# CycloneBoy/pdf_table

Measured on AMD Instinct MI355X. Metric: pages/s, higher is better.
Workload: dtype bf16

## Files before the change

include/pdftable_hip.h:

```cpp
#ifndef PDFTABLE_HIP_H
#define PDFTABLE_HIP_H

#include <stddef.h>
#include <stdint.h>

#ifdef __cplusplus
extern "C" {
#endif

#define PT_OK 0
#define PT_ERR_INVALID 1
#define PT_ERR_HIP 2
#define PT_ERR_STATE 3
#define PT_ERR_FORMAT 4

typedef struct pt_engine pt_engine;
typedef void* pt_stream;

int pt_engine_create(int device_id, pt_engine** out);
void pt_engine_destroy(pt_engine* e);
const char* pt_last_error(void);
int pt_abi_version(void);
int pt_engine_check(pt_engine* e);
int pt_engine_set_lstm_cluster(pt_engine* e, int on);
// ... 121 lines not shown
  int32_t resized_w;
  int32_t img_w;
  int32_t reserved;
  int64_t out_off;
} pt_rec_pp_item;
int pt_rec_pp_preprocess(pt_engine* e, const uint8_t* d_pages_rgb, int n_pages, int h, int w, const pt_rec_line* d_lines,
                         const int64_t* h_crop_px, int n_lines, const pt_rec_pp_item* d_items, int n_items, int img_h,
                         int max_img_w, float* d_out, pt_stream stream);
int pt_rec_pp_preprocess_crops(pt_engine* e, const uint8_t* d_crops_rgb, const pt_rec_line* d_lines, const int64_t* h_crop_px,
                               int n_lines, const pt_rec_pp_item* d_items, int n_items, int img_h, int max_img_w, float* d_out,
                               pt_stream stream);

typedef struct pt_tsr_table {
  double minv[6];
  int32_t page, x0, y0, crop_w, crop_h, reserved;
} pt_tsr_table;

int pt_tsr_preprocess(pt_engine* e, const uint8_t* d_pages_rgb, int n_pages, int ph, int pw, const pt_tsr_table* d_tables,
                      int n, int inp_h, int inp_w, int bgr, uint16_t* d_out_bf16, pt_stream stream);

#define PT_TSR_CS_SMALL 8
#define PT_TSR_CS_FEAT 256
int pt_tsr_forward_net(pt_engine* e, const uint16_t* d_input_bf16, int n, int H, int W, float* d_hm, float* d_st,
                       float* d_wh, float* d_ax, float* d_cr, float* d_reg, pt_stream stream);

int pt_tsr_forward_net_wireless(pt_engine* e, const uint16_t* d_input_bf16, int n, int H, int W, float* d_hm, float* d_st,
                                float* d_wh, float* d_ax, float* d_cr, float* d_reg, pt_stream stream);

#define PT_TSR_MAX_CELLS 3000
int pt_tsr_decode(pt_engine* e, const float* d_hm, const float* d_st, const float* d_wh, const float* d_ax,
                  const float* d_cr, const float* d_reg, int n, int h, int w, int wiz_rev, float vis_thresh,
                  int32_t* d_counts, float* d_dets, float* d_logi, pt_stream stream);

int pt_tsr_forward_decode(pt_engine* e, const uint16_t* d_input_bf16, int n, int in_h, int in_w, int wiz_rev,
                          float vis_thresh, int32_t* d_counts, float* d_dets, float* d_logi, pt_stream stream);

int pt_centernet_forward_net(pt_engine* e, const uint16_t* d_input_bf16, int n, int H, int W, float* d_hm, float* d_v2c, float* d_c2v,
                             float* d_reg, pt_stream stream);

#define PT_CENTERNET_MAX_CELLS 1000
int pt_centernet_decode(pt_engine* e, const float* d_hm, const float* d_v2c, const float* d_c2v, const float* d_reg, int n, int h, int w,
                        const double* d_affine, int32_t* d_counts, float* d_cells, pt_stream stream);

int pt_tsr_process(pt_engine* e, const float* d_logi, const float* d_dets, const int32_t* h_counts, int n_tables,
                   int use_2dpe, float* d_logic, float* d_stacked, pt_stream stream);

int pt_op_conv2d(pt_engine* e, const uint16_t* d_in, int B, int H, int W, int Cin, const uint16_t* d_w_tiled,
                 const float* d_bias, int N, int ks, int stride, uint16_t* d_out, int out_cstride, int out_coff,
                 int rep, int shuffle_cout, const uint16_t* d_res, int res_mode, int relu, int split, int out_lo_off,
                 pt_stream stream);
int pt_op_conv1x1_ex(pt_engine* e, const uint16_t* d_in, int B, int H, int W, int Cin, const uint16_t* d_w_tiled, const float* d_bias,
                     int N, uint16_t* d_out, float* d_out_f32, int out_cstride, int n_valid, const float* d_res_f32, int relu,
                     const int32_t* d_ylimit, pt_stream stream);

int pt_op_dcn(pt_engine* e, const uint16_t* d_in, const float* d_om, int B, int H, int W, int C, const uint16_t* d_w_tiled,
              const float* d_bias, int N, uint16_t* d_out, int relu, int split, pt_stream stream);

int pt_op_dwconvt_up_add(pt_engine* e, const uint16_t* d_in, const float* d_w, const uint16_t* d_add, uint16_t* d_out, int B, int h, int w, int C,
                         int f, int split, pt_stream stream);
int pt_op_dcn_up_add(pt_engine* e, const uint16_t* d_in, const float* d_om, int B, int H, int W, int C, const uint16_t* d_w_tiled,
                     const float* d_bias, int N, uint16_t* d_out, int relu, int split, const uint16_t* d_up_in, int up_h, int up_w,
                     const float* d_up_w, int up_f, pt_stream stream);

int pt_op_stem7x7(pt_engine* e, const uint16_t* d_in, int B, int H, int W, const uint16_t* d_w, const float* d_bias,
                  uint16_t* d_out, int split, pt_stream stream);
int pt_op_maxpool3x3s2(pt_engine* e, const uint16_t* d_in, int B, int H, int W, int C, uint16_t* d_out, int split,
                       pt_stream stream);
int pt_op_db_head_final(pt_engine* e, const uint16_t* d_in, int B, int H, int W, const void* d_w, const float* d_bias,
                        float* d_prob, float* d_logits, int split, pt_stream stream);

int pt_op_dwconv(pt_engine* e, const uint16_t* d_in, int B, int H, int W, int C, const float* d_w_taps, const float* d_bias, int k,
                 int stride, int act, uint16_t* d_out, int split, pt_stream stream);
int pt_op_add(pt_engine* e, const uint16_t* d_a, const uint16_t* d_b, uint16_t* d_out, long long npix, int C, int split, pt_stream stream);
int pt_op_maxpool(pt_engine* e, const uint16_t* d_in, int B, int H, int W, int C, int k, int stride, int pad, uint16_t* d_out,
                  int split, pt_stream stream);
int pt_op_avgpool(pt_engine* e, const uint16_t* d_in, int B, int H, int W, int C, int k, uint16_t* d_out, int split, pt_stream stream);
int pt_op_chan_mean(pt_engine* e, const uint16_t* d_in, int B, int HW, int C, float* d_scratch, uint16_t* d_mean, int split, pt_stream stream);
int pt_op_chan_mean_scratch_floats(int B, int C);
int pt_op_scale_channels(pt_engine* e, const uint16_t* d_in, const uint16_t* d_gate, int B, int HW, int C, uint16_t* d_out,
                         int split, pt_stream stream);
int pt_op_act(pt_engine* e, const uint16_t* d_in, long long n_elems, int kind, float alpha, float beta, uint16_t* d_out, int C, int split,
              pt_stream stream);
int pt_op_copy_channels(pt_engine* e, const uint16_t* d_src, long long npix, int src_cstride, int src_coff, uint16_t* d_dst, int dst_cstride, int dst_coff,
                        int n, pt_stream stream);
int pt_op_upsample_nearest(pt_engine* e, const uint16_t* d_in, int B, int H, int W, int C, int factor, uint16_t* d_out, pt_stream stream);
int pt_op_mul(pt_engine* e, const uint16_t* d_a, const uint16_t* d_b, uint16_t* d_out, long long n_elems, int C, int split, pt_stream stream);
int pt_copy_bytes(pt_engine* e, const void* src, void* dst, long long nbytes, pt_stream stream);
int pt_op_layernorm(pt_engine* e, const uint16_t* d_in, long long rows, int c_pad, int c, const float* d_gamma, const float* d_beta, float eps,
                    uint16_t* d_out, int split, pt_stream stream);
int pt_op_softmax(pt_engine* e, const uint16_t* d_in, long long rows, int c_pad, int c, float* d_out_f32, uint16_t* d_out_bf16, int split, pt_stream stream);
int pt_op_attention(pt_engine* e, const uint16_t* d_qkv, int B, int T, int heads, int d, int qkv_cstride, float scale, uint16_t* d_out, int out_cstride,
                    int split, pt_stream stream);

int pt_op_lstm(pt_engine* e, const uint16_t* d_pregates, int pg_cstride, const uint16_t* d_r_packed, int T, int B, int H, int dirs, int reverse,
               uint16_t* d_y, int y_cstride, int split, pt_stream stream);
int pt_op_lstm_packed_elems(int H, int dirs, int split);

int pt_op_conv2d_rect(pt_engine* e, const uint16_t* d_in, int B, int H, int W, int Cin, const uint16_t* d_w_tiled, const float* d_bias, int N, int kh,
                      int kw, int sh, int sw, uint16_t* d_out, int out_cstride, int out_coff, int act, int split, int out_lo_off, pt_stream stream);
int pt_op_dwconv_rect(pt_engine* e, const uint16_t* d_in, int B, int H, int W, int C, const float* d_w_taps, const float* d_bias, int k, int sh, int sw,
                      int act, uint16_t* d_out, int split, pt_stream stream);
int pt_op_pool_rect(pt_engine* e, const uint16_t* d_in, int B, int H, int W, int C, int kind, int kh, int kw, uint16_t* d_out, int split,
                    pt_stream stream);

int pt_op_affine_act(pt_engine* e, const uint16_t* d_in, long long npix, int Cpad, int C, const float* d_s1, const float* d_b1, const float* d_s2,
                     const float* d_b2, int act, uint16_t* d_out, int split, pt_stream stream);
// ... 61 lines not shown
```

pdf_table_amd/csrc/c_api.hip:

```cpp
#include <stdarg.h>
#include <stdio.h>
#include <stdlib.h>

#include <cmath>

#include "common.h"

namespace PT_FMT_NS {
namespace api {

static int ensure(void** buf, size_t* cap, size_t need);

int pt_engine_check(pt_engine* e) {
  PT_REQUIRE(e, "pt_engine_check: null engine");
  if (e->lstm_err && *e->lstm_err) {
    *e->lstm_err = 0;
    e->lstm_cluster = 0;
    pt_set_error("lstm_cluster_kernel: a workgroup waited > 2^22 polls for its peers -- the launch was not co-resident "
                 "(GPU shared with another process or stream?).  The recognition results since the last check are invalid; "
                 "this engine now uses the streaming LSTM kernel (pt_engine_set_lstm_cluster(e, 0)): run the batch again");
    return PT_ERR_HIP;
  }
  return PT_OK;
}
// ... 880 lines not shown

int pt_cls_forward_lines_direct(pt_engine* e, int slot, const uint8_t* d_pages_rgb, int n_pages, int h, int w, const pt_rec_line* d_lines,
                                int n_lines, int max_crop_h, int max_crop_w, int out_h, int out_w, int textline, float* d_logits,
                                int* n_classes, pt_stream stream) {
  PT_REQUIRE(e && d_pages_rgb && d_lines && d_logits && n_lines > 0 && n_pages > 0 && h > 0 && w > 0,
             "pt_cls_forward_lines_direct: bad arguments");
  PT_HIP_CHECK(hipSetDevice(e->device));
  hipStream_t s = reinterpret_cast<hipStream_t>(stream);
  int rc;
  if ((rc = cls_lut(e)) != PT_OK) return rc;
  const int mb = cls_microbatch(), x3 = pt_split(e);
  const size_t per = (size_t)out_h * out_w * (x3 ? 8 : 4);
  const int cap = mb < n_lines ? mb : n_lines;
  if ((rc = ensure(&e->cls_direct_in, &e->cls_direct_in_cap, (size_t)cap * per * sizeof(bf16_t))) != PT_OK) return rc;
  bf16_t* xin = reinterpret_cast<bf16_t*>(e->cls_direct_in);
  for (int i0 = 0; i0 < n_lines; i0 += mb) {
    const int nb = (n_lines - i0) < mb ? (n_lines - i0) : mb;
    {
      PtProfScope ps(e, s, PT_PROF_OTHER, 0, "cls line resize+norm");
      rc = pt_launch_cls_line_resize_norm(d_pages_rgb, h, w, d_lines + i0, nb, max_crop_h, max_crop_w, out_h, out_w, e->cls_lut, x3, xin, s);
      if (rc != PT_OK) return rc;
    }
    rc = pt_pplcnet_forward_net(e, slot, xin, nb, out_h, out_w, textline, d_logits + (size_t)i0 * PT_CLS_MAX_CLASSES, n_classes, s,
                                PT_ARENA_CLS);
    if (rc != PT_OK) return rc;
  }
  return PT_OK;
}

int pt_op_conv2d(pt_engine* e, const uint16_t* d_in, int B, int H, int W, int Cin, const uint16_t* d_w_tiled,
                 const float* d_bias, int N, int ks, int stride, uint16_t* d_out, int out_cstride, int out_coff,
                 int rep, int shuffle_cout, const uint16_t* d_res, int res_mode, int relu, int split, int out_lo_off,
                 pt_stream stream) {
  PT_REQUIRE(e != nullptr, "pt_op_conv2d: null engine");
  ConvDesc d;
  d.in = d_in; d.B = B; d.H = H; d.W = W; d.Cin = Cin; d.w = d_w_tiled; d.bias = d_bias; d.N = N; d.ks = ks;
  d.stride = stride; d.out = d_out; d.out_cstride = out_cstride; d.out_coff = out_coff; d.rep = rep;
  d.shuffle_cout = shuffle_cout; d.res = d_res; d.res_mode = res_mode; d.relu = relu;
  d.split = split; d.out_lo_off = out_lo_off;
  return pt_launch_conv(e, d, reinterpret_cast<hipStream_t>(stream));
}

int pt_op_conv1x1_ex(pt_engine* e, const uint16_t* d_in, int B, int H, int W, int Cin, const uint16_t* d_w_tiled, const float* d_bias,
                     int N, uint16_t* d_out, float* d_out_f32, int out_cstride, int n_valid, const float* d_res_f32, int relu,
                     const int32_t* d_ylimit, pt_stream stream) {
  PT_REQUIRE(e != nullptr, "pt_op_conv1x1_ex: null engine");
  ConvDesc d;
  d.in = d_in; d.B = B; d.H = H; d.W = W; d.Cin = Cin; d.w = d_w_tiled; d.bias = d_bias; d.N = N; d.ks = 1; d.stride = 1;
  d.out = d_out_f32 ? nullptr : d_out; d.out_f32 = d_out_f32; d.out_cstride = out_cstride; d.n_valid = n_valid; d.res_f32 = d_res_f32;
  d.relu = relu; d.ylimit = d_ylimit;
  return pt_launch_conv(e, d, reinterpret_cast<hipStream_t>(stream));
}

int pt_op_stem7x7(pt_engine* e, const uint16_t* d_in, int B, int H, int W, const uint16_t* d_w, const float* d_bias,
                  uint16_t* d_out, int split, pt_stream stream) {
  PT_REQUIRE(e != nullptr, "pt_op_stem7x7: null engine");
  return pt_launch_stem7x7(e, d_in, B, H, W, d_w, d_bias, d_out, split, reinterpret_cast<hipStream_t>(stream));
}

int pt_op_maxpool3x3s2(pt_engine* e, const uint16_t* d_in, int B, int H, int W, int C, uint16_t* d_out, int split,
                       pt_stream stream) {
  PT_REQUIRE(e && d_in && d_out, "pt_op_maxpool3x3s2: bad arguments");
  return pt_launch_maxpool3x3s2(d_in, B, H, W, C, d_out, split, reinterpret_cast<hipStream_t>(stream));
}

int pt_op_db_head_final(pt_engine* e, const uint16_t* d_in, int B, int H, int W, const void* d_w, const float* d_bias,
                        float* d_prob, float* d_logits, int split, pt_stream stream) {
  PT_REQUIRE(e && d_in && d_w && d_bias && (d_prob || d_logits), "pt_op_db_head_final: bad arguments");
  return pt_launch_db_head_final(d_in, B, H, W, d_w, d_bias, d_prob, d_logits, split, reinterpret_cast<hipStream_t>(stream));
}

int pt_op_dcn(pt_engine* e, const uint16_t* d_in, const float* d_om, int B, int H, int W, int C, const uint16_t* d_w_tiled,
              const float* d_bias, int N, uint16_t* d_out, int relu, int split, pt_stream stream) {
  PT_REQUIRE(e && d_in && d_om && d_w_tiled && d_bias && d_out, "pt_op_dcn: null argument");
  PT_REQUIRE(B > 0 && H > 0 && W > 0, "pt_op_dcn: empty map (B=%d H=%d W=%d)", B, H, W);
  return pt_launch_dcn_fused(e, d_in, d_om, d_w_tiled, d_bias, d_out, B, H, W, C, N, split, relu, reinterpret_cast<hipStream_t>(stream));
}

int pt_op_dwconvt_up_add(pt_engine* e, const uint16_t* d_in, const float* d_w, const uint16_t* d_add, uint16_t* d_out, int B, int h, int w, int C,
                         int f, int split, pt_stream stream) {
  PT_REQUIRE(e && d_in && d_w && d_out, "pt_op_dwconvt_up_add: null argument");
  PT_REQUIRE(B > 0 && h > 0 && w > 0 && C > 0, "pt_op_dwconvt_up_add: empty map (B=%d h=%d w=%d C=%d)", B, h, w, C);
  return pt_launch_dwconvt_up_add(d_in, d_w, d_add, d_out, B, h, w, C, f, split, reinterpret_cast<hipStream_t>(stream));
}

int pt_op_dcn_up_add(pt_engine* e, const uint16_t* d_in, const float* d_om, int B, int H, int W, int C, const uint16_t* d_w_tiled,
                     const float* d_bias, int N, uint16_t* d_out, int relu, int split, const uint16_t* d_up_in, int up_h, int up_w,
                     const float* d_up_w, int up_f, pt_stream stream) {
  PT_REQUIRE(e && d_in && d_om && d_w_tiled && d_bias && d_out && d_up_in && d_up_w, "pt_op_dcn_up_add: null argument");
  PT_REQUIRE(B > 0 && H > 0 && W > 0, "pt_op_dcn_up_add: empty map (B=%d H=%d W=%d)", B, H, W);
  PT_REQUIRE(split == 0, "pt_op_dcn_up_add: the (hi | lo) modes keep the two launches (pt_op_dcn, pt_op_dwconvt_up_add)");
  PT_REQUIRE((up_f == 2 || up_f == 4) && up_h > 0 && up_w > 0 && up_h * up_f == H && up_w * up_f == W,
             "pt_op_dcn_up_add: a %dx%d map times %d is not the %dx%d output", up_h, up_w, up_f, H, W);
  return pt_launch_dcn_fused(e, d_in, d_om, d_w_tiled, d_bias, d_out, B, H, W, C, N, split, relu, reinterpret_cast<hipStream_t>(stream), nullptr, nullptr,
                             d_up_in, d_up_w, up_f);
}

int pt_profile_enable(pt_engine* e, int on) {
  PT_REQUIRE(e != nullptr, "pt_profile_enable: null engine");
  PT_REQUIRE(on >= 0 && on < 2 + PT_PROF_NCLASS, "pt_profile_enable: mode %d out of range", on);
  if (on && !e->prof.h_lims)
    PT_HIP_CHECK(hipHostMalloc(reinterpret_cast<void**>(&e->prof.h_lims), PtProfile::MAX_LIMS * sizeof(int), hipHostMallocDefault));
  e->prof.on = on;
  return PT_OK;
}

// ... 75 lines not shown
```

pdf_table_amd/csrc/rec_kernels.hip:

```cpp
#include <math.h>

#include "common.h"

namespace PT_FMT_NS {

typedef __attribute__((ext_vector_type(8))) __bf16 bf16x8;
typedef __attribute__((ext_vector_type(16))) float f32x16;
typedef __attribute__((ext_vector_type(4))) uint32_t u32x4;
typedef __attribute__((ext_vector_type(2))) uint32_t u32x2;

__device__ __forceinline__ float rbf2f(uint32_t bits16) { return a16_to_f32(bits16); }
__device__ __forceinline__ uint32_t rf2bf(float f) { return f32_to_a16(f); }

__global__ __launch_bounds__(256) void rec_warp_kernel(const uint8_t* __restrict__ pages, int ph, int pw,
                                                        const pt_rec_line* __restrict__ lines, int n_lines,
                                                        const long long* __restrict__ pix_off, uint8_t* __restrict__ crops) {
  a16_kernel_enter();
  const int li = blockIdx.y;
  if (li >= n_lines) return;
  const pt_rec_line L = lines[li];
  const int cw = L.crop_w, chh = L.crop_h;
  const long long npx = (long long)cw * chh;
  uint8_t* dst = crops + pix_off[li] * 3;
  const uint8_t* src = pages + (size_t)L.page * ph * pw * 3;
// ... 1847 lines not shown
    hipLaunchKernelGGL((gemm_argmax_kernel<32, 0, 8>), dim3((unsigned)((M + 255) / 256)), dim3(512), SMEM, s, A, M, W3, bias, N, ids, rowmax, nullptr, 0,
                       nullptr, 2 * K, wts);
  }
  if (cls_dma())
    hipLaunchKernelGGL(cls_argmax_dma_kernel<1>, dim3((unsigned)((M + 255) / 256)), dim3(512), CLS_DMA_SMEM, s, A, M, W3, bias, N, nullptr, nullptr, 2 * K, wts,
                       reinterpret_cast<const float*>(wmax), rowmax, cand);
  else
    hipLaunchKernelGGL((gemm_cand_kernel<32>), dim3((unsigned)((M + 127) / 128)), dim3(256), SMEM, s, A, M, 2 * K, W3, wts, bias, N,
                       reinterpret_cast<const float*>(wmax), rowmax, cand);
  hipLaunchKernelGGL(cand_eval_kernel, dim3((unsigned)((M + 15) / 16)), dim3(256), 0, s, A, M, 2 * K, K, W3, bias, N, n_real, cand, ids, maxv, ovf_count,
                     ovf_rows);
  hipLaunchKernelGGL(cand_full_kernel, dim3(2048), dim3(256), 0, s, A, 2 * K, K, W3, bias, n_real, ovf_count, ovf_rows, ids, maxv);
  PT_HIP_CHECK(hipGetLastError());
  return PT_OK;
}

static int gemm_nw(int dflt) {
  static int nw = -1;
  if (nw < 0) {
    const char* ev = getenv("PT_GEMM_NW");
    nw = ev ? (atoi(ev) == 8 ? 8 : 4) : 0;
  }
  return nw ? nw : dflt;
}

int pt_launch_gemm_argmax(const bf16_t* A, long long M, int K, const bf16_t* W, const float* bias, int N, int* ids, float* maxv,
                          hipStream_t s) {
  if ((K != 512 && K != 192) || N % 64 != 0 || M <= 0) return PT_ERR_INVALID;
  constexpr int SMEM = 64 * (512 * 2 + 16) + 64 * 4;
  static bool attr_done = false;
  if (!attr_done) {
    PT_HIP_CHECK(hipFuncSetAttribute(reinterpret_cast<const void*>(&gemm_argmax_kernel<32, 0>), hipFuncAttributeMaxDynamicSharedMemorySize, SMEM));
    PT_HIP_CHECK(hipFuncSetAttribute(reinterpret_cast<const void*>(&gemm_argmax_kernel<12, 0>), hipFuncAttributeMaxDynamicSharedMemorySize, SMEM));
    PT_HIP_CHECK(hipFuncSetAttribute(reinterpret_cast<const void*>(&gemm_argmax_kernel<32, 0, 8>), hipFuncAttributeMaxDynamicSharedMemorySize, SMEM));
    PT_HIP_CHECK(hipFuncSetAttribute(reinterpret_cast<const void*>(&gemm_argmax_kernel<12, 0, 8>), hipFuncAttributeMaxDynamicSharedMemorySize, SMEM));
    attr_done = true;
  }
  const int nw = gemm_nw(K == 512 ? 8 : 4);
  const dim3 grid((unsigned)((M + nw * 32 - 1) / (nw * 32))), blk(nw * 64);
  if (K == 192) {
    if (nw == 8) hipLaunchKernelGGL((gemm_argmax_kernel<12, 0, 8>), grid, blk, 64 * (192 * 2 + 16) + 64 * 4, s, A, M, W, bias, N, ids, maxv, nullptr, 0, nullptr, 192, 6ll * 2048);
    else hipLaunchKernelGGL((gemm_argmax_kernel<12, 0>), grid, blk, 64 * (192 * 2 + 16) + 64 * 4, s, A, M, W, bias, N, ids, maxv, nullptr, 0, nullptr, 192, 6ll * 2048);
  } else {
    if (nw == 8 && cls_dma()) {
      if (cls_dma_attr() != PT_OK) return PT_ERR_HIP;
      hipLaunchKernelGGL(cls_argmax_dma_kernel<0>, grid, blk, CLS_DMA_SMEM, s, A, M, W, bias, N, ids, maxv, 512, 16ll * 2048, nullptr, nullptr, nullptr);
    } else if (nw == 8) hipLaunchKernelGGL((gemm_argmax_kernel<32, 0, 8>), grid, blk, SMEM, s, A, M, W, bias, N, ids, maxv, nullptr, 0, nullptr, 512, 16ll * 2048);
    else hipLaunchKernelGGL((gemm_argmax_kernel<32, 0>), grid, blk, SMEM, s, A, M, W, bias, N, ids, maxv, nullptr, 0, nullptr, 512, 16ll * 2048);
  }
  PT_HIP_CHECK(hipGetLastError());
  return PT_OK;
}

int pt_launch_gemm_rows(const bf16_t* A, long long M, int K, const bf16_t* W, const float* bias, int N, bf16_t* out, int relu,
                        hipStream_t s, const int* tlim) {
  if ((K != 512 && K != 256) || N % 64 != 0 || M <= 0) return PT_ERR_INVALID;
  const int nw = gemm_nw(4);
  const int smem = 64 * (K * 2 + 16) + 64 * 4 + nw * 32 * 80;
  static bool attr_done = false;
  if (!attr_done) {
    PT_HIP_CHECK(hipFuncSetAttribute(reinterpret_cast<const void*>(&gemm_argmax_kernel<32, 1>), hipFuncAttributeMaxDynamicSharedMemorySize, 64 * (512 * 2 + 16) + 256 + 4 * 32 * 80));
    PT_HIP_CHECK(hipFuncSetAttribute(reinterpret_cast<const void*>(&gemm_argmax_kernel<32, 1, 8>), hipFuncAttributeMaxDynamicSharedMemorySize, 64 * (512 * 2 + 16) + 256 + 8 * 32 * 80));
    attr_done = true;
  }
  const dim3 grid((unsigned)((M + nw * 32 - 1) / (nw * 32))), blk(nw * 64);
  if (K == 512) {
    if (nw == 8) hipLaunchKernelGGL((gemm_argmax_kernel<32, 1, 8>), grid, blk, smem, s, A, M, W, bias, N, nullptr, nullptr, out, relu, tlim, 512, 16ll * 2048);
    else hipLaunchKernelGGL((gemm_argmax_kernel<32, 1>), grid, blk, smem, s, A, M, W, bias, N, nullptr, nullptr, out, relu, tlim, 512, 16ll * 2048);
  } else {
    if (nw == 8) hipLaunchKernelGGL((gemm_argmax_kernel<16, 1, 8>), grid, blk, smem, s, A, M, W, bias, N, nullptr, nullptr, out, relu, tlim, 256, 8ll * 2048);
    else hipLaunchKernelGGL((gemm_argmax_kernel<16, 1>), grid, blk, smem, s, A, M, W, bias, N, nullptr, nullptr, out, relu, tlim, 256, 8ll * 2048);
  }
  PT_HIP_CHECK(hipGetLastError());
  return PT_OK;
}

template <int KSTEPS>
__global__ __launch_bounds__(256, KSTEPS == 32 ? 1 : 2) void gemm_rows_x3_kernel(const bf16_t* __restrict__ A, long long M, const bf16_t* __restrict__ W3,
                                                                                 const float* __restrict__ bias, int N, bf16_t* __restrict__ out, int relu,
                                                                                 const int* __restrict__ tlim) {
  a16_kernel_enter();
  constexpr int K = KSTEPS * 16, NCH = K / 32, P = K * 2 + 16;
  constexpr int NPF = NCH;
  extern __shared__ __attribute__((aligned(16))) char smem[];
  char* sw = smem;
  float* sb = reinterpret_cast<float*>(smem + 64 * P);
  const int tid = threadIdx.x, lane = tid & 63, wave = tid >> 6;
  const int lx = lane & 31, q = lane >> 5;
  long long row0 = ((long long)blockIdx.x * 4 + wave) * 32;
  bool live = row0 < M;
  if (tlim) {
    const int total = tlim[0], g = blockIdx.x * 4 + wave;
    if ((int)blockIdx.x * 4 >= total) return;
    live = g < total;
    row0 = live ? (long long)tlim[1 + g] * 32 : 0;
  }
  const long long row = row0 + lx;
  const long long rc = row < M ? row : M - 1;
  bf16x8 ahi[KSTEPS], alo[KSTEPS];
#pragma unroll
  for (int ks = 0; ks < KSTEPS; ++ks) {
    ahi[ks] = *reinterpret_cast<const bf16x8*>(A + rc * (2 * K) + ks * 16 + q * 8);
    alo[ks] = *reinterpret_cast<const bf16x8*>(A + rc * (2 * K) + K + ks * 16 + q * 8);
  }
  u32x4 pf[NPF];
  float pb = 0.f;
  auto prefetch = [&](int st) {
    const bf16_t* wt = W3 + (size_t)(st >> 1) * (3 * NCH * 2048) + (st & 1) * (32 * 32);
#pragma unroll
    for (int j = 0; j < NPF; ++j) {
      const int idx = tid + j * 256, plane = idx / (NCH * 128), rem = idx - plane * (NCH * 128), c = rem >> 7, rp = rem & 127;
      pf[j] = *reinterpret_cast<const u32x4*>(wt + (size_t)(plane * 2 * NCH + c) * 2048 + rp * 8);
    }
    if (tid < 32) pb = bias[st * 32 + tid];
  };
  auto commit = [&]() {
// ... 95 lines not shown
```

pdf_table_amd/engine.py:

```python
from __future__ import annotations

import contextlib
import ctypes as C
import functools
import threading
from typing import Optional, Sequence, Tuple

import numpy as np
import torch

from . import lib as L

__all__ = ["HipEngine", "REC_LINE_DTYPE", "CLS_IMAGE_DTYPE", "REC_PP_ITEM_DTYPE"]

TSR_TABLE_DTYPE = np.dtype([("minv", "<f8", (6,)), ("page", "<i4"), ("x0", "<i4"), ("y0", "<i4"),
                            ("crop_w", "<i4"), ("crop_h", "<i4"), ("reserved", "<i4")])
CLS_IMAGE_DTYPE = np.dtype([("offset", "<i8"), ("h", "<i4"), ("w", "<i4")])
REC_LINE_DTYPE = np.dtype([("minv", np.float64, (9,)), ("page", np.int32), ("crop_w", np.int32), ("crop_h", np.int32),
                           ("reserved", np.int32)])


REC_PP_ITEM_DTYPE = np.dtype([("line", "<i4"), ("resized_w", "<i4"), ("img_w", "<i4"), ("reserved", "<i4"),
                              ("out_off", "<i8")])

# ... 576 lines not shown
        T, Tc = cfg["max_len"] + 1, cfg["max_len_cell"] + 1
        tag = torch.zeros((n, T, cfg["num_classes"]), dtype=torch.float32, device=self._tdev)
        box = torch.zeros((n, T, 4), dtype=torch.float32, device=self._tdev)
        lens = np.zeros(n, np.int32)
        counts = np.zeros(n, np.int32)
        ip = lambda a: a.ctypes.data_as(C.POINTER(C.c_int))
        L.check(self.lib.pt_tsr_mtl_structure(self._h, _ptr(f3), n, hw, _ptr(tag), _ptr(box), ip(lens), ip(counts), 1 if force_redecode else 0,
                                              self._stream()), "pt_tsr_mtl_structure")
        total = int(counts.sum())
        steps = np.zeros(n, np.int32)
        ids = torch.zeros((max(total, 1), Tc), dtype=torch.int32, device=self._tdev)
        prob = torch.zeros((max(total, 1), Tc), dtype=torch.float32, device=self._tdev)
        logits = torch.zeros((max(total, 1), Tc, cfg["num_classes_cell"]), dtype=torch.float32, device=self._tdev) if want_cell_logits else None
        L.check(self.lib.pt_tsr_mtl_cells(self._h, total, _ptr(ids), _ptr(prob), _ptr(logits), ip(steps), 1 if force_redecode else 0, self._stream()),
                "pt_tsr_mtl_cells")
        return dict(tag_logits=tag, boxes=box, lens=lens, cell_counts=counts, cell_steps=steps, cell_ids=ids[:total], cell_prob=prob[:total],
                    cell_logits=None if logits is None else logits[:total], cfg=cfg)

    def op_conv2d(self, x: torch.Tensor, w_tiled: torch.Tensor, bias: torch.Tensor, ks: int, stride: int = 1,
                  relu: bool = False, res: Optional[torch.Tensor] = None, res_mode: int = 0, rep: int = 1,
                  shuffle_cout: int = 0, out: Optional[torch.Tensor] = None, out_coff: int = 0,
                  split: int = 0) -> torch.Tensor:
        self._chk(x, self.act_dtype, "x")
        self._chk(bias, torch.float32, "bias")
        B, H, W, Cin = x.shape
        m = 2 if split else 1
        Cin //= m
        N = bias.numel()
        pad = ks // 2
        Ho, Wo = (H + 2 * pad - ks) // stride + 1, (W + 2 * pad - ks) // stride + 1
        if out is None:
            if shuffle_cout:
                out = torch.empty((B, 2 * Ho, 2 * Wo, shuffle_cout * m), dtype=self.act_dtype, device=self._tdev)
            else:
                out = torch.empty((B, Ho * rep, Wo * rep, N * m), dtype=self.act_dtype, device=self._tdev)
        L.check(self.lib.pt_op_conv2d(self._h, _ptr(x), B, H, W, Cin, _ptr(w_tiled), _ptr(bias), N, ks, stride,
                                      _ptr(out), out.shape[-1], out_coff, rep, shuffle_cout, _ptr(res), res_mode,
                                      int(relu), int(split), out.shape[-1] // 2, self._stream()), "pt_op_conv2d")
        return out

    def op_conv1x1_ex(self, x: torch.Tensor, w_tiled: torch.Tensor, bias: torch.Tensor, relu: int = 0, out_f32: bool = False,
                      n_valid: int = 0, res_f32: Optional[torch.Tensor] = None, ylimit: Optional[torch.Tensor] = None) -> torch.Tensor:
        self._chk(x, self.act_dtype, "x")
        self._chk(bias, torch.float32, "bias")
        B, H, W, Cin = x.shape
        N = bias.numel()
        cs = n_valid or N
        out = torch.zeros((B, H, W, cs), dtype=torch.float32 if out_f32 else self.act_dtype, device=self._tdev)
        L.check(self.lib.pt_op_conv1x1_ex(self._h, _ptr(x), B, H, W, Cin, _ptr(w_tiled), _ptr(bias), N, None if out_f32 else _ptr(out),
                                          _ptr(out) if out_f32 else None, cs, n_valid, _ptr(res_f32), int(relu), _ptr(ylimit),
                                          self._stream()), "pt_op_conv1x1_ex")
        return out

    def op_dcn(self, x: torch.Tensor, om: torch.Tensor, w_tiled: torch.Tensor, bias: torch.Tensor, relu: bool = True, split: int = 0) -> torch.Tensor:
        self._chk(x, self.act_dtype, "x")
        self._chk(om, torch.float32, "om")
        self._chk(bias, torch.float32, "bias")
        B, H, W, Cc = x.shape
        m = 2 if split else 1
        Cc //= m
        if tuple(om.shape) != (B, H, W, 32):
            raise ValueError(f"op_dcn: om must be [B,H,W,32], got {tuple(om.shape)}")
        N = bias.numel()
        out = torch.empty((B, H, W, N * m), dtype=self.act_dtype, device=self._tdev)
        L.check(self.lib.pt_op_dcn(self._h, _ptr(x), _ptr(om), B, H, W, Cc, _ptr(w_tiled), _ptr(bias), N, _ptr(out), int(relu), int(split),
                                   self._stream()), "pt_op_dcn")
        return out

    def op_dwconvt_up_add(self, x: torch.Tensor, w_taps: torch.Tensor, add: Optional[torch.Tensor], f: int, split: int = 0) -> torch.Tensor:
        self._chk(x, self.act_dtype, "x")
        self._chk(w_taps, torch.float32, "w_taps")
        B, h, w, Cc = x.shape
        if add is not None:
            self._chk(add, self.act_dtype, "add")
            if tuple(add.shape) != (B, h * f, w * f, Cc):
                raise ValueError(f"op_dwconvt_up_add: add must be {(B, h * f, w * f, Cc)}, got {tuple(add.shape)}")
        out = torch.empty((B, h * f, w * f, Cc), dtype=self.act_dtype, device=self._tdev)
        L.check(self.lib.pt_op_dwconvt_up_add(self._h, _ptr(x), _ptr(w_taps), _ptr(add), _ptr(out), B, h, w, Cc // 2 if split else Cc, int(f),
                                              int(split), self._stream()), "pt_op_dwconvt_up_add")
        return out

    def op_dcn_up_add(self, x: torch.Tensor, om: torch.Tensor, w_tiled: torch.Tensor, bias: torch.Tensor, up_in: torch.Tensor, up_taps: torch.Tensor,
                      f: int, relu: bool = True, split: int = 0) -> torch.Tensor:
        self._chk(x, self.act_dtype, "x")
        self._chk(om, torch.float32, "om")
        self._chk(bias, torch.float32, "bias")
        self._chk(up_in, self.act_dtype, "up_in")
        self._chk(up_taps, torch.float32, "up_taps")
        B, H, W, Cc = x.shape
        if tuple(om.shape) != (B, H, W, 32):
            raise ValueError(f"op_dcn_up_add: om must be [B,H,W,32], got {tuple(om.shape)}")
        N = bias.numel()
        if up_in.dim() != 4 or up_in.shape[0] != B or up_in.shape[3] != N:
            raise ValueError(f"op_dcn_up_add: up_in must be [{B},h,w,{N}], got {tuple(up_in.shape)}")
        out = torch.empty((B, H, W, N), dtype=self.act_dtype, device=self._tdev)
        L.check(self.lib.pt_op_dcn_up_add(self._h, _ptr(x), _ptr(om), B, H, W, Cc // 2 if split else Cc, _ptr(w_tiled), _ptr(bias), N, _ptr(out), int(relu),
                                          int(split), _ptr(up_in), up_in.shape[1], up_in.shape[2], _ptr(up_taps), int(f), self._stream()),
                "pt_op_dcn_up_add")
        return out

    def op_dwconv(self, x: torch.Tensor, w_taps: torch.Tensor, bias: torch.Tensor, k: int, stride: int = 1, act: int = 0, split: bool = False) -> torch.Tensor:
        self._chk(x, self.act_dtype, "x")
        self._chk(w_taps, torch.float32, "w_taps")
        self._chk(bias, torch.float32, "bias")
        B, H, W, Cc = x.shape
        pad = k // 2
# ... 341 lines not shown
```

pdf_table_amd/lib.py:

```python
from __future__ import annotations

import ctypes as C
import os

_HERE = os.path.dirname(os.path.abspath(__file__))
LIB_PATH = os.environ.get("PT_LIB_PATH") or os.path.join(_HERE, "libpdftable_hip.so")

PT_MODEL_DB_RESNET18 = 1
PT_MODEL_CRNN = 2
PT_MODEL_LORE_DLA34 = 3
PT_MODEL_LORE_PROCESSOR = 4
PT_MODEL_PICODET = 5
PT_MODEL_LORE_RESNET18 = 6
PT_MODEL_DB_NAS = 7
PT_MODEL_PPLCNET = 8
PT_MODEL_CONVNEXT_VIT = 16
PT_MODEL_MTL_BACKBONE = 17
PT_MODEL_MTL_DECODER = 18
PT_MODEL_CENTERNET_DLA34 = 19
PT_CVIT_W, PT_CVIT_CHUNK_W, PT_CVIT_CHUNK_STEP, PT_CVIT_T, PT_CVIT_NCLS = 804, 300, 252, 201, 7644
PT_CLS_SLOTS = 4
PT_CLS_MAX_CLASSES = 16
PT_LAYOUT_HEAD_CS, PT_LAYOUT_CAND_FLOATS = 40, 48
PT_DET_PRE_DB_PP = 0
# ... 36 lines not shown
        "pt_weights_load_device": (i, [vp, i, vp, sz, vp]),
        "pt_det_plan": (i, [i, i, i, ip, ip]),
        "pt_det_forward": (i, [vp, vp, i, i, i, i, f, i, vp, vp, vp]),
        "pt_det_forward_net": (i, [vp, vp, i, i, i, vp, vp, vp]),
        "pt_det_preprocess": (i, [vp, vp, i, i, i, i, vp, vp]),
        "pt_det_bitmap": (i, [vp, vp, i, i, i, f, i, vp, vp]),
        "pt_det_box_scores": (i, [vp, vp, i, i, i, vp, i, vp, vp]),
        "pt_db_candidates": (i, [vp, i, i, i, f, vp, vp, i, ip]),
        "pt_db_finalize": (i, [vp, vp, i, f, f, f, i, i, i, i, i, vp, vp, i, ip]),
        "pt_db_candidates_batch": (i, [vp, i, i, i, i, f, i, vp, vp, i, vp]),
        "pt_db_finalize_batch": (i, [vp, vp, vp, i, i, f, f, f, i, i, i, i, i, i, i, vp, vp, vp, vp]),
        "pt_rec_forward": (i, [vp, vp, i, i, i, vp, vp, i, vp, vp, vp]),
        "pt_rec_forward_crops": (i, [vp, vp, vp, vp, i, vp, vp, vp]),
        "pt_rec_forward_net": (i, [vp, vp, i, vp, vp, vp]),
        "pt_rec_preprocess": (i, [vp, vp, i, i, i, vp, vp, i, vp, vp]),
        "pt_rec_cvit_forward": (i, [vp, vp, i, i, i, vp, vp, vp, i, vp, vp, vp]),
        "pt_rec_cvit_forward_crops": (i, [vp, vp, vp, vp, vp, i, vp, vp, vp]),
        "pt_rec_cvit_forward_net": (i, [vp, vp, i, i, vp, vp, vp, vp]),
        "pt_rec_cvit_preprocess_crops": (i, [vp, vp, vp, vp, i, vp, vp]),
        "pt_tsr_mtl_backbone_net": (i, [vp, vp, i, i, i, vp, vp]),
        "pt_tsr_mtl_preprocess": (i, [vp, vp, i, i, i, vp, i, i, vp, vp]),
        "pt_tsr_mtl_resized_size": (None, [i, i, i, ip, ip]),
        "pt_tsr_mtl_decoder_config": (i, [vp, ip]),
        "pt_tsr_mtl_structure": (i, [vp, vp, i, i, vp, vp, ip, ip, i, vp]),
        "pt_tsr_mtl_cells": (i, [vp, i, vp, vp, vp, ip, i, vp]),
        "pt_rec_pp_preprocess": (i, [vp, vp, i, i, i, vp, vp, i, vp, i, i, i, vp, vp]),
        "pt_rec_pp_preprocess_crops": (i, [vp, vp, vp, vp, i, vp, i, i, i, vp, vp]),
        "pt_layout_plan": (i, [i, i, ip, ip]),
        "pt_layout_preprocess": (i, [vp, vp, i, i, i, i, i, vp, vp]),
        "pt_layout_forward_net": (i, [vp, vp, i, i, i, vp, vp, vp, vp, vp]),
        "pt_layout_candidates": (i, [vp, vp, vp, vp, vp, i, i, i, i, f, i, vp, vp, vp]),
        "pt_layout_forward": (i, [vp, vp, i, i, i, i, i, i, f, i, vp, vp, vp]),
        "pt_tsr_preprocess": (i, [vp, vp, i, i, i, vp, i, i, i, i, vp, vp]),
        "pt_tsr_forward_net": (i, [vp, vp, i, i, i, vp, vp, vp, vp, vp, vp, vp]),
        "pt_tsr_forward_net_wireless": (i, [vp, vp, i, i, i, vp, vp, vp, vp, vp, vp, vp]),
        "pt_tsr_decode": (i, [vp, vp, vp, vp, vp, vp, vp, i, i, i, i, f, vp, vp, vp, vp]),
        "pt_tsr_forward_decode": (i, [vp, vp, i, i, i, i, f, vp, vp, vp, vp]),
        "pt_tsr_process": (i, [vp, vp, vp, vp, i, i, vp, vp, vp]),
        "pt_centernet_forward_net": (i, [vp, vp, i, i, i, vp, vp, vp, vp, vp]),
        "pt_centernet_decode": (i, [vp, vp, vp, vp, vp, i, i, i, vp, vp, vp, vp]),
        "pt_hard_nms": (i, [vp, vp, vp, i, C.c_double, i, vp, vp]),
        "pt_page_line_mask": (i, [vp, i, i, i, vp, vp]),
        "pt_page_line_angles": (i, [vp, i, i, i, i, i, vp, i, vp]),
        "pt_page_warp_cubic": (i, [vp, i, i, i, vp, vp, i, vp, vp]),
        "pt_page_quarter_turn": (i, [vp, i, i, i, i, vp, vp]),
        "pt_page_pre_tables": (i, [vp, vp]),
        "pt_cls_preprocess": (i, [vp, vp, vp, i, i, i, i, i, vp, vp]),
        "pt_cls_forward_net": (i, [vp, i, vp, i, i, i, i, vp, ip, vp]),
        "pt_cls_forward": (i, [vp, i, vp, vp, i, i, i, i, i, i, vp, ip, vp]),
        "pt_cls_forward_lines": (i, [vp, i, vp, i, i, i, vp, vp, i, i, i, i, i, i, vp, ip, vp]),
        "pt_cls_forward_lines_direct": (i, [vp, i, vp, i, i, i, vp, i, i, i, i, i, i, vp, ip, vp]),
        "pt_op_conv2d": (i, [vp, vp, i, i, i, i, vp, vp, i, i, i, vp, i, i, i, i, vp, i, i, i, i, vp]),
        "pt_op_conv1x1_ex": (i, [vp, vp, i, i, i, i, vp, vp, i, vp, vp, i, i, vp, i, vp, vp]),
        "pt_op_dcn": (i, [vp, vp, vp, i, i, i, i, vp, vp, i, vp, i, i, vp]),
        "pt_op_dwconvt_up_add": (i, [vp, vp, vp, vp, vp, i, i, i, i, i, i, vp]),
        "pt_op_dcn_up_add": (i, [vp, vp, vp, i, i, i, i, vp, vp, i, vp, i, i, vp, i, i, vp, i, vp]),
        "pt_op_stem7x7": (i, [vp, vp, i, i, i, vp, vp, vp, i, vp]),
        "pt_op_maxpool3x3s2": (i, [vp, vp, i, i, i, i, vp, i, vp]),
        "pt_op_db_head_final": (i, [vp, vp, i, i, i, vp, vp, vp, vp, i, vp]),
        "pt_op_dwconv": (i, [vp, vp, i, i, i, i, vp, vp, i, i, i, vp, i, vp]),
        "pt_op_add": (i, [vp, vp, vp, vp, C.c_longlong, i, i, vp]),
        "pt_op_maxpool": (i, [vp, vp, i, i, i, i, i, i, i, vp, i, vp]),
        "pt_op_avgpool": (i, [vp, vp, i, i, i, i, i, vp, i, vp]),
        "pt_op_chan_mean": (i, [vp, vp, i, i, i, vp, vp, i, vp]),
        "pt_op_chan_mean_scratch_floats": (i, [i, i]),
        "pt_op_scale_channels": (i, [vp, vp, vp, i, i, i, vp, i, vp]),
        "pt_op_act": (i, [vp, vp, C.c_longlong, i, C.c_float, C.c_float, vp, i, i, vp]),
        "pt_op_copy_channels": (i, [vp, vp, C.c_longlong, i, i, vp, i, i, i, vp]),
        "pt_op_upsample_nearest": (i, [vp, vp, i, i, i, i, i, vp, vp]),
        "pt_op_mul": (i, [vp, vp, vp, vp, C.c_longlong, i, i, vp]),
        "pt_copy_bytes": (i, [vp, vp, vp, C.c_longlong, vp]),
        "pt_op_layernorm": (i, [vp, vp, C.c_longlong, i, i, vp, vp, C.c_float, vp, i, vp]),
        "pt_op_softmax": (i, [vp, vp, C.c_longlong, i, i, vp, vp, i, vp]),
        "pt_op_attention": (i, [vp, vp, i, i, i, i, i, C.c_float, vp, i, i, vp]),
        "pt_op_lstm": (i, [vp, vp, i, vp, i, i, i, i, i, vp, i, i, vp]),
        "pt_op_lstm_packed_elems": (i, [i, i, i]),
        "pt_op_conv2d_rect": (i, [vp, vp, i, i, i, i, vp, vp, i, i, i, i, i, vp, i, i, i, i, i, vp]),
        "pt_op_dwconv_rect": (i, [vp, vp, i, i, i, i, vp, vp, i, i, i, i, vp, i, vp]),
        "pt_op_pool_rect": (i, [vp, vp, i, i, i, i, i, i, i, vp, i, vp]),
        "pt_op_affine_act": (i, [vp, vp, C.c_longlong, i, i, vp, vp, vp, vp, i, vp, i, vp]),
        "pt_op_db_tail": (i, [vp, vp, i, i, i, i, i, i, vp, vp, vp, vp, vp, i, vp]),
        "pt_profile_enable": (i, [vp, i]),
        "pt_profile_read": (i, [vp, vp, vp, vp]),
        "pt_profile_read_labels": (i, [vp, C.c_char_p, i]),
    }
    for name, (res, args) in P.items():
        try:
            fn = getattr(lib, name)
        except AttributeError:
            raise PtError(f"{LIB_PATH} does not export {name}: it was built from older sources; rebuild it (`python -m pdf_table_amd.build --force`)") from None
        fn.restype = res
        fn.argtypes = args
    return P


EXPORTS = None


def load():
    global _lib, EXPORTS
    if _lib is None:
        import torch
        if not os.path.exists(LIB_PATH):
            raise PtError(f"{LIB_PATH} not found: run `python -m pdf_table_amd.build` (hipcc, gfx950). "
                          "There is no CPU fallback.")
        lib = C.CDLL(LIB_PATH, mode=C.RTLD_GLOBAL)
# ... 14 lines not shown
```

Measured before the change: 787.6.

## Add DMA-pipelined K=256 row GEMM kernel with LDS-staged weight tiles

Adds a new rows_dma_kernel for K=256 row GEMMs that keeps A rows in registers, streams 64-column weight tiles into LDS with buffer_load_lds DMA double-buffering, and interleaves MFMA with the next tile's loads using scheduling barriers. Outputs go through an LDS transpose tile so each store is a coalesced 128-bit buffer store. It is enabled by default unless PT_ROWS_DMA=0, and a pt_op_gemm_rows C/Python entry point is exposed for it. The aim is to hide weight-fetch latency and raise MFMA utilization. In exchange it needs large LDS and runs one 512-thread block per CU, which could limit occupancy.

```diff
diff --git a/include/pdftable_hip.h b/include/pdftable_hip.h
--- a/include/pdftable_hip.h
+++ b/include/pdftable_hip.h
@@ -197,6 +197,9 @@
 int pt_op_conv1x1_ex(pt_engine* e, const uint16_t* d_in, int B, int H, int W, int Cin, const uint16_t* d_w_tiled, const float* d_bias,
                      int N, uint16_t* d_out, float* d_out_f32, int out_cstride, int n_valid, const float* d_res_f32, int relu,
                      const int32_t* d_ylimit, pt_stream stream);
+
+int pt_op_gemm_rows(pt_engine* e, const uint16_t* d_a, long long M, int K, const uint16_t* d_w_tiled, const float* d_bias, int N,
+                    uint16_t* d_out, int relu, const int32_t* d_live, pt_stream stream);
 
 int pt_op_dcn(pt_engine* e, const uint16_t* d_in, const float* d_om, int B, int H, int W, int C, const uint16_t* d_w_tiled,
               const float* d_bias, int N, uint16_t* d_out, int relu, int split, pt_stream stream);
diff --git a/pdf_table_amd/csrc/c_api.hip b/pdf_table_amd/csrc/c_api.hip
--- a/pdf_table_amd/csrc/c_api.hip
+++ b/pdf_table_amd/csrc/c_api.hip
@@ -956,6 +956,14 @@
   return pt_launch_conv(e, d, reinterpret_cast<hipStream_t>(stream));
 }
 
+int pt_op_gemm_rows(pt_engine* e, const uint16_t* d_a, long long M, int K, const uint16_t* d_w_tiled, const float* d_bias, int N,
+                    uint16_t* d_out, int relu, const int32_t* d_live, pt_stream stream) {
+  PT_REQUIRE(e != nullptr, "pt_op_gemm_rows: null engine");
+  PT_REQUIRE(e->precision == PT_PRECISION_BF16 || e->precision == PT_PRECISION_F16, "pt_op_gemm_rows: single-pass precisions only");
+  PT_REQUIRE(relu == 0 || relu == 1 || relu == 4, "pt_op_gemm_rows: relu must be 0, 1 or 4");
+  return pt_launch_gemm_rows(d_a, M, K, d_w_tiled, d_bias, N, d_out, relu, reinterpret_cast<hipStream_t>(stream), d_live);
+}
+
 int pt_op_stem7x7(pt_engine* e, const uint16_t* d_in, int B, int H, int W, const uint16_t* d_w, const float* d_bias,
                   uint16_t* d_out, int split, pt_stream stream) {
   PT_REQUIRE(e != nullptr, "pt_op_stem7x7: null engine");
diff --git a/pdf_table_amd/csrc/rec_kernels.hip b/pdf_table_amd/csrc/rec_kernels.hip
--- a/pdf_table_amd/csrc/rec_kernels.hip
+++ b/pdf_table_amd/csrc/rec_kernels.hip
@@ -1923,6 +1923,165 @@
   return PT_OK;
 }
 
+template <int ACT>
+__device__ __forceinline__ void rows_tile_to_lds(const f32x16& acc, const float* bs, char* dst) {
+#pragma unroll
+  for (int rg = 0; rg < 4; ++rg) {
+    const a16_f32x4 b4 = *reinterpret_cast<const a16_f32x4*>(bs + rg * 8);
+    uint32_t hb[4];
+#pragma unroll
+    for (int k = 0; k < 4; ++k) {
+      float v = acc[rg * 4 + k] + b4[k];
+      if (ACT == 1) v = fmaxf(v, 0.f);
+      else if (ACT == 4) v = gelu_poly(v);
+      hb[k] = rf2bf(v);
+    }
+    *reinterpret_cast<u32x2*>(dst + rg * 16) = u32x2{hb[0] | (hb[1] << 16), hb[2] | (hb[3] << 16)};
+  }
+}
+
+constexpr int ROWS_DMA_SMEM = 2 * 32 * (1024 + 16) + 2 * 64 * 4 + 8 * 32 * 144;
+
+__global__ __launch_bounds__(512, 1) void rows_dma_kernel(const bf16_t* __restrict__ A, long long M, const bf16_t* __restrict__ W,
+                                                          const float* __restrict__ bias, int N, bf16_t* __restrict__ out, int relu,
+                                                          const int* __restrict__ tlim) {
+#if defined(__HIP_DEVICE_COMPILE__)
+  a16_kernel_enter();
+  constexpr int NW = 8, KSTEPS = 16, K = 256, BLK = 1024 + 16, TILE = 32 * BLK, D = 2;
+  constexpr int NDMA = 32 / NW, EVERY = 2 * KSTEPS / NDMA;
+  constexpr int TP = 128 + 16;
+  extern __shared__ __attribute__((aligned(16))) char smem[];
+  float* sb = reinterpret_cast<float*>(smem + 2 * TILE);
+  const int tid = threadIdx.x, lane = tid & 63;
+  const int wave = __builtin_amdgcn_readfirstlane(tid >> 6);
+  const int lx = lane & 31, q = lane >> 5;
+  char* tile = smem + 2 * TILE + 512 + wave * (32 * TP);
+  const long long g0 = ((long long)blockIdx.x * NW + wave) * 2;
+  long long row0[2];
+  bool live[2];
+  if (tlim) {
+    const int total = tlim[0];
+    if ((long long)blockIdx.x * NW * 2 >= total) return;
+#pragma unroll
+    for (int i = 0; i < 2; ++i) {
+      live[i] = g0 + i < total;
+      row0[i] = live[i] ? (long long)tlim[1 + g0 + i] * 32 : 0;
+    }
+  } else {
+#pragma unroll
+    for (int i = 0; i < 2; ++i) {
+      row0[i] = (g0 + i) * 32;
+      live[i] = row0[i] < M;
+    }
+  }
+  bf16x8 areg[2][KSTEPS];
+#pragma unroll
+  for (int i = 0; i < 2; ++i) {
+    const long long row = row0[i] + lx;
+    const long long rc = row < M ? row : M - 1;
+#pragma unroll
+    for (int ks = 0; ks < KSTEPS; ++ks) areg[i][ks] = *reinterpret_cast<const bf16x8*>(A + rc * K + ks * 16 + q * 8);
+  }
+  constexpr int OOB = 0x7FFFF000;
+  const __amdgpu_buffer_rsrc_t r_w = __builtin_amdgcn_make_buffer_rsrc(const_cast<bf16_t*>(W), 0, OOB, 0x00020000);
+  int voff[NDMA];
+  {
+    const int i = lane >> 5, p = (lane & 31) ^ (8 * i);
+#pragma unroll
+    for (int s = 0; s < NDMA; ++s) voff[s] = ((((p >> 2) * 64 + 2 * (wave + NW * s) + i) * 32) + (p & 3) * 8) * 2;
+  }
+  const int fbase = (lx >> 1) * BLK + (lx & 1) * 512 + q * 16;
+  const int fa = fbase + (lx & 1) * 128, fb = fbase - (lx & 1) * 128;
+  const int NT = N / 64;
+#pragma unroll
+  for (int s = 0; s < NDMA; ++s)
+    __builtin_amdgcn_raw_ptr_buffer_load_lds(r_w, (__attribute__((address_space(3))) void*)(smem + (wave + NW * s) * BLK), 16, voff[s], 0, 0, 0);
+  if (tid < 64) sb[tid] = bias[tid];
+  float pb = tid < 64 ? bias[(NT > 1 ? 64 : 0) + tid] : 0.f;
+#pragma unroll
+  for (int i = 0; i < 2; ++i)
+#pragma unroll
+    for (int ks = 0; ks < KSTEPS; ++ks) asm volatile("" : "+v"(areg[i][ks]));
+  __amdgpu_buffer_rsrc_t r_o[2];
+#pragma unroll
+  for (int i = 0; i < 2; ++i) {
+    const long long left = M - row0[i];
+    const int nrec = !live[i] || left <= 0 ? 0 : (int)(left < 32 ? left : 32) * N * 2;
+    r_o[i] = __builtin_amdgcn_make_buffer_rsrc(out + row0[i] * N, 0, __builtin_amdgcn_readfirstlane(nrec), 0x00020000);
+  }
+  constexpr int NST = 8;
+  asm volatile("s_waitcnt vmcnt(0)" ::: "memory");
+  for (int t = 0; t < NT; ++t) {
+    const int b = t & 1;
+    __syncthreads();
+    const bool more = t + 1 < NT;
+    const int soff = more ? (t + 1) * (K * 64 * 2) : 0;
+    if (tid < 64) {
+      sb[(b ^ 1) * 64 + tid] = pb;
+      pb = bias[(t + 2 < NT ? t + 2 : t) * 64 + tid];
+    }
+    const float* sbt = sb + b * 64;
+    f32x16 acc[2][2];
+#pragma unroll
+    for (int half = 0; half < 2; ++half) {
+      const char* wa = smem + b * TILE + half * 16 * BLK + fa;
+      const char* wb = smem + b * TILE + half * 16 * BLK + fb;
+#pragma unroll
+      for (int r = 0; r < 16; ++r) { acc[half][0][r] = 0.f; acc[half][1][r] = 0.f; }
+      bf16x8 f[D + 1];
+#pragma unroll
+      for (int d = 0; d < D; ++d) f[d] = *reinterpret_cast<const bf16x8*>(wa + d * 32);
+#pragma unroll
+      for (int ks = 0; ks < KSTEPS; ++ks) {
+        if (ks + D < KSTEPS) f[(ks + D) % (D + 1)] = *reinterpret_cast<const bf16x8*>((((ks + D) & 4) ? wb : wa) + (ks + D) * 32);
+        acc[half][0] = mfma_32x32x16_a16(f[ks % (D + 1)], areg[0][ks], acc[half][0]);
+        acc[half][1] = mfma_32x32x16_a16(f[ks % (D + 1)], areg[1][ks], acc[half][1]);
+        if ((half * KSTEPS + ks) % EVERY == 0) {
+          const int s = (half * KSTEPS + ks) / EVERY;
+          __builtin_amdgcn_raw_ptr_buffer_load_lds(r_w, (__attribute__((address_space(3))) void*)(smem + (b ^ 1) * TILE + (wave + NW * s) * BLK), 16,
+                                                   more ? voff[s] : OOB, soff, 0, 0);
+        }
+      }
+      __builtin_amdgcn_sched_group_barrier(0x100, D, 0);
+#pragma unroll
+      for (int ks = 0; ks < KSTEPS; ++ks) {
+        __builtin_amdgcn_sched_group_barrier(0x008, 1, 0);
+        if (ks + D < KSTEPS) __builtin_amdgcn_sched_group_barrier(0x100, 1, 0);
+        __builtin_amdgcn_sched_group_barrier(0x008, 1, 0);
+        if ((half * KSTEPS + ks) % EVERY == 0) __builtin_amdgcn_sched_group_barrier(0x020, 1, 0);
+      }
+      __builtin_amdgcn_sched_barrier(0);
+    }
+#pragma unroll
+    for (int i = 0; i < 2; ++i) {
+#pragma unroll
+      for (int h = 0; h < 2; ++h) {
+        const float* bs = sbt + h * 32 + 4 * q;
+        char* dst = tile + lx * TP + h * 64 + q * 8;
+        if (relu == 4) rows_tile_to_lds<4>(acc[h][i], bs, dst);
+        else if (relu == 1) rows_tile_to_lds<1>(acc[h][i], bs, dst);
+        else rows_tile_to_lds<0>(acc[h][i], bs, dst);
+      }
+      asm volatile("s_waitcnt lgkmcnt(0)" ::: "memory");
+#pragma unroll
+      for (int j = 0; j < 4; ++j) {
+        const int r = (lane >> 3) + 8 * j;
+        const u32x4 v = *reinterpret_cast<const u32x4*>(tile + r * TP + (lane & 7) * 16);
+        __builtin_amdgcn_raw_buffer_store_b128(v, r_o[i], (r * N + t * 64 + (lane & 7) * 8) * 2, 0, 0);
+      }
+      asm volatile("s_waitcnt lgkmcnt(0)" ::: "memory");
+    }
+    __builtin_amdgcn_sched_barrier(0);
+    asm volatile("s_waitcnt vmcnt(%0)" ::"n"(NST) : "memory");
+  }
+#endif
+}
+
+static bool rows_dma() {
+  const char* ev = getenv("PT_ROWS_DMA");
+  return !(ev && ev[0] == '0');
+}
+
 int pt_launch_gemm_rows(const bf16_t* A, long long M, int K, const bf16_t* W, const float* bias, int N, bf16_t* out, int relu,
                         hipStream_t s, const int* tlim) {
   if ((K != 512 && K != 256) || N % 64 != 0 || M <= 0) return PT_ERR_INVALID;
@@ -1933,6 +2092,16 @@
     PT_HIP_CHECK(hipFuncSetAttribute(reinterpret_cast<const void*>(&gemm_argmax_kernel<32, 1>), hipFuncAttributeMaxDynamicSharedMemorySize, 64 * (512 * 2 + 16) + 256 + 4 * 32 * 80));
     PT_HIP_CHECK(hipFuncSetAttribute(reinterpret_cast<const void*>(&gemm_argmax_kernel<32, 1, 8>), hipFuncAttributeMaxDynamicSharedMemorySize, 64 * (512 * 2 + 16) + 256 + 8 * 32 * 80));
     attr_done = true;
+  }
+  if (K == 256 && rows_dma()) {
+    static bool dma_attr_done = false;
+    if (!dma_attr_done) {
+      PT_HIP_CHECK(hipFuncSetAttribute(reinterpret_cast<const void*>(&rows_dma_kernel), hipFuncAttributeMaxDynamicSharedMemorySize, ROWS_DMA_SMEM));
+      dma_attr_done = true;
+    }
+    hipLaunchKernelGGL(rows_dma_kernel, dim3((unsigned)((M + 511) / 512)), dim3(512), ROWS_DMA_SMEM, s, A, M, W, bias, N, out, relu, tlim);
+    PT_HIP_CHECK(hipGetLastError());
+    return PT_OK;
   }
   const dim3 grid((unsigned)((M + nw * 32 - 1) / (nw * 32))), blk(nw * 64);
   if (K == 512) {
diff --git a/pdf_table_amd/engine.py b/pdf_table_amd/engine.py
--- a/pdf_table_amd/engine.py
+++ b/pdf_table_amd/engine.py
@@ -652,6 +652,18 @@
                                           self._stream()), "pt_op_conv1x1_ex")
         return out
 
+    def op_gemm_rows(self, a: torch.Tensor, w_tiled: torch.Tensor, bias: torch.Tensor, relu: int = 0, live: Optional[torch.Tensor] = None) -> torch.Tensor:
+        self._chk(a, self.act_dtype, "a")
+        self._chk(bias, torch.float32, "bias")
+        if live is not None:
+            self._chk(live, torch.int32, "live")
+        M, K = a.shape
+        N = bias.numel()
+        out = torch.zeros((M, N), dtype=self.act_dtype, device=self._tdev)
+        L.check(self.lib.pt_op_gemm_rows(self._h, _ptr(a), M, K, _ptr(w_tiled), _ptr(bias), N, _ptr(out), int(relu), _ptr(live), self._stream()),
+                "pt_op_gemm_rows")
+        return out
+
     def op_dcn(self, x: torch.Tensor, om: torch.Tensor, w_tiled: torch.Tensor, bias: torch.Tensor, relu: bool = True, split: int = 0) -> torch.Tensor:
         self._chk(x, self.act_dtype, "x")
         self._chk(om, torch.float32, "om")
diff --git a/pdf_table_amd/lib.py b/pdf_table_amd/lib.py
--- a/pdf_table_amd/lib.py
+++ b/pdf_table_amd/lib.py
@@ -112,6 +112,7 @@
         "pt_cls_forward_lines_direct": (i, [vp, i, vp, i, i, i, vp, i, i, i, i, i, i, vp, ip, vp]),
         "pt_op_conv2d": (i, [vp, vp, i, i, i, i, vp, vp, i, i, i, vp, i, i, i, i, vp, i, i, i, i, vp]),
         "pt_op_conv1x1_ex": (i, [vp, vp, i, i, i, i, vp, vp, i, vp, vp, i, i, vp, i, vp, vp]),
+        "pt_op_gemm_rows": (i, [vp, vp, C.c_longlong, i, vp, vp, i, vp, i, vp, vp]),
         "pt_op_dcn": (i, [vp, vp, vp, i, i, i, i, vp, vp, i, vp, i, i, vp]),
         "pt_op_dwconvt_up_add": (i, [vp, vp, vp, vp, vp, i, i, i, i, i, i, vp]),
         "pt_op_dcn_up_add": (i, [vp, vp, vp, i, i, i, i, vp, vp, i, vp, i, i, vp, i, i, vp, i, vp]),
```

Result: no change. 785.9, median of 2 (-0.2%).
